# google/speedy

Measured on AMD Instinct MI355X. Metric: Msamples/s processed (16 kHz mono, 3.5x nonlinear), higher is better.
Workload: dtype int16 samples; f64 DFT, f32 features, int32 AMDF/OLA

## Files before the change

include/speedy_hip.h:

```cpp
#ifndef SPEEDY_HIP_H_
#define SPEEDY_HIP_H_
#include <stddef.h>
#include <stdint.h>
#ifdef __cplusplus
extern "C" {
#endif

#ifndef SPX_FEATURE_COUNT
#define SPX_FEATURE_COUNT 15
#endif

typedef struct spx_plan* spx_plan_t;

typedef struct {
  int64_t in_off;
  int64_t n_in;
  int64_t out_off;
  int64_t out_cap;
  int32_t channels;
  float speed;
  float nonlinear;
  float feedback;
} spx_stream_job;

// ... 52 lines not shown
void* spx_host_alloc(size_t bytes);
void spx_host_free(void* p);

int spx_batch_analyze(spx_plan_t plan, const spx_stream_job* jobs, int n_streams, const int16_t* in,
                      void* workspace, size_t workspace_bytes, const spx_taps* taps, void* hip_stream);
int spx_batch_walk(spx_plan_t plan, const spx_stream_job* jobs, int n_streams, const int16_t* in,
                   int16_t* out, int64_t* n_out, void* workspace, size_t workspace_bytes,
                   const spx_taps* taps, void* hip_stream);

size_t spx_batch_workspace_bytes_mixed(const spx_plan_t* plans, int n_plans, const spx_stream_job* jobs,
                                       const int* plan_index, int n_streams);
int spx_batch_run_mixed(const spx_plan_t* plans, int n_plans, const spx_stream_job* jobs, const int* plan_index,
                        int n_streams, const int16_t* in, int16_t* out, int64_t* n_out, void* workspace,
                        size_t workspace_bytes, void* hip_stream);

int spx_batch_run_mixed_taps(const spx_plan_t* plans, int n_plans, const spx_stream_job* jobs, const int* plan_index,
                             int n_streams, const int16_t* in, int16_t* out, int64_t* n_out, void* workspace,
                             size_t workspace_bytes, const spx_taps* taps, void* hip_stream);
int spx_batch_run_mixed_ahead(const spx_plan_t* plans, int n_plans, const spx_stream_job* jobs, const int* plan_index,
                              int n_streams, const int16_t* in, int16_t* out, int64_t* n_out, void* workspace,
                              size_t workspace_bytes, void* hip_stream);

void spx_set_timing(int enabled);
void spx_set_pipeline_chunks(int chunks);
void spx_set_concurrent(int on);
int spx_timing_collect(double* sum_ms_analyze, double* sum_ms_walk, int* n_calls);
const char* spx_batch_kernel_names(spx_plan_t plan, int n_streams, int max_channels, int speedup_only);
const char* spx_batch_kernel_names_lean(spx_plan_t plan, int n_streams, int max_channels, int speedup_only);
int spx_debug_last_walk_form(void);
int spx_debug_kernel_vgprs(int which);
int spx_debug_walk_info(int sample_rate, int channels, int n_streams, int speedup_only, int short_jobs, int lean, int* out5);
int spx_debug_analysis_info(int sample_rate, int* out4);
int spx_debug_mode_resources(int sample_rate, int channels, int n_streams, int speedup_only, long long* out22);
long long spx_debug_fdiv_check(unsigned seed, unsigned denominators, int exp_lo, int exp_hi);
long long spx_debug_xfade_check(int n_lo, int n_hi);
long long spx_debug_arith_check(unsigned seed, unsigned threads, unsigned per_thread);
int spx_debug_log_check(unsigned first_block, unsigned end_block, unsigned long long* sums);
int spx_debug_last_call_concurrent(void);
double spx_timing_last_tension_ms(void);

int spx_batch_read_steps(spx_plan_t plan, const spx_stream_job* jobs, int n_streams, const void* workspace,
                         int32_t* steps, void* hip_stream);
int spx_batch_read_steps_mixed(const spx_plan_t* plans, int n_plans, const spx_stream_job* jobs, const int* plan_index,
                               int n_streams, const void* workspace, int32_t* steps, void* hip_stream);

void* spx_device_alloc(size_t bytes);
void spx_device_free(void* p);
int spx_batch_pack_outputs(const spx_stream_job* jobs, int n_streams, const int16_t* out, const int64_t* n_out,
                           int16_t* packed, int64_t* offsets, void* hip_stream);
int spx_copy_to_device(void* dst, const void* src, size_t bytes, void* hip_stream);
int spx_copy_to_host(void* dst, const void* src, size_t bytes, void* hip_stream);
int spx_stream_synchronize(void* hip_stream);

#ifdef __cplusplus
}
#endif
#endif
```

speedy_amd/_lib.py:

```python
import ctypes as C
import os
import subprocess

_HERE = os.path.dirname(os.path.abspath(__file__))
LIB_PATH = os.environ.get("SPEEDY_HIP_LIB") or os.path.join(_HERE, "lib", "libspeedy_hip.so")
_LIB = None

c_short_p = C.POINTER(C.c_short)
c_float_p = C.POINTER(C.c_float)
c_int64_p = C.POINTER(C.c_int64)


class StreamJob(C.Structure):
    _fields_ = [("in_off", C.c_int64), ("n_in", C.c_int64), ("out_off", C.c_int64), ("out_cap", C.c_int64),
                ("channels", C.c_int32), ("speed", C.c_float), ("nonlinear", C.c_float), ("feedback", C.c_float)]


class Taps(C.Structure):
    _fields_ = [("tension", C.c_void_p), ("speed", C.c_void_p), ("features", C.c_void_p),
                ("spectrogram", C.c_void_p), ("normalized", C.c_void_p)]


TENSION_FN = C.CFUNCTYPE(None, C.c_void_p, C.c_int, C.c_float)
FEATURES_FN = C.CFUNCTYPE(None, C.c_void_p, C.c_int, c_float_p)
# ... 21 lines not shown
    "spx_batch_run_ahead_when": (C.c_int, [C.c_void_p, C.POINTER(StreamJob), C.c_int, C.c_void_p, C.c_void_p, C.c_void_p,
                                           C.c_void_p, C.c_size_t, C.POINTER(Taps), C.c_void_p, C.c_void_p]),
    "spx_batch_workspace_bytes_mixed": (C.c_size_t, [C.POINTER(C.c_void_p), C.c_int, C.POINTER(StreamJob), C.POINTER(C.c_int), C.c_int]),
    "spx_batch_run_mixed": (C.c_int, [C.POINTER(C.c_void_p), C.c_int, C.POINTER(StreamJob), C.POINTER(C.c_int), C.c_int,
                                      C.c_void_p, C.c_void_p, C.c_void_p, C.c_void_p, C.c_size_t, C.c_void_p]),
    "spx_batch_run_mixed_ahead": (C.c_int, [C.POINTER(C.c_void_p), C.c_int, C.POINTER(StreamJob), C.POINTER(C.c_int), C.c_int,
                                      C.c_void_p, C.c_void_p, C.c_void_p, C.c_void_p, C.c_size_t, C.c_void_p]),
    "spx_batch_run_mixed_taps": (C.c_int, [C.POINTER(C.c_void_p), C.c_int, C.POINTER(StreamJob), C.POINTER(C.c_int), C.c_int,
                                           C.c_void_p, C.c_void_p, C.c_void_p, C.c_void_p, C.c_size_t, C.POINTER(Taps), C.c_void_p]),
    "spx_batch_read_steps": (C.c_int, [C.c_void_p, C.POINTER(StreamJob), C.c_int, C.c_void_p, C.POINTER(C.c_int32), C.c_void_p]),
    "spx_batch_read_steps_mixed": (C.c_int, [C.POINTER(C.c_void_p), C.c_int, C.POINTER(StreamJob), C.POINTER(C.c_int), C.c_int,
                                             C.c_void_p, C.POINTER(C.c_int32), C.c_void_p]),
    "spx_batch_analyze": (C.c_int, [C.c_void_p, C.POINTER(StreamJob), C.c_int, C.c_void_p, C.c_void_p,
                                    C.c_size_t, C.POINTER(Taps), C.c_void_p]),
    "spx_batch_walk": (C.c_int, [C.c_void_p, C.POINTER(StreamJob), C.c_int, C.c_void_p, C.c_void_p, C.c_void_p,
                                 C.c_void_p, C.c_size_t, C.POINTER(Taps), C.c_void_p]),
    "spx_set_timing": (None, [C.c_int]),
    "spx_set_pipeline_chunks": (None, [C.c_int]),
    "spx_set_concurrent": (None, [C.c_int]),
    "spx_timing_collect": (C.c_int, [C.POINTER(C.c_double), C.POINTER(C.c_double), C.POINTER(C.c_int)]),
    "spx_timing_last_tension_ms": (C.c_double, []),
    "spx_batch_kernel_names": (C.c_char_p, [C.c_void_p, C.c_int, C.c_int, C.c_int]),
    "spx_batch_kernel_names_lean": (C.c_char_p, [C.c_void_p, C.c_int, C.c_int, C.c_int]),
    "spx_debug_last_walk_form": (C.c_int, []),
    "spx_debug_kernel_vgprs": (C.c_int, [C.c_int]),
    "spx_debug_last_call_concurrent": (C.c_int, []),
    "spx_debug_fdiv_check": (C.c_longlong, [C.c_uint, C.c_uint, C.c_int, C.c_int]),
    "spx_debug_xfade_check": (C.c_longlong, [C.c_int, C.c_int]),
    "spx_debug_arith_check": (C.c_longlong, [C.c_uint, C.c_uint, C.c_uint]),
    "spx_debug_log_check": (C.c_int, [C.c_uint, C.c_uint, C.POINTER(C.c_ulonglong)]),
    "spx_debug_walk_info": (C.c_int, [C.c_int, C.c_int, C.c_int, C.c_int, C.c_int, C.c_int, C.POINTER(C.c_int)]),
    "spx_debug_analysis_info": (C.c_int, [C.c_int, C.POINTER(C.c_int)]),
    "spx_debug_mode_resources": (C.c_int, [C.c_int, C.c_int, C.c_int, C.c_int, C.POINTER(C.c_longlong)]),
    "spx_pipeline_create": (C.c_void_p, [C.c_void_p, C.POINTER(StreamJob), C.c_int, C.c_int, C.c_uint]),
    "spx_pipeline_create_mixed": (C.c_void_p, [C.POINTER(C.c_void_p), C.c_int, C.POINTER(StreamJob), C.POINTER(C.c_int), C.c_int, C.c_int, C.c_uint]),
    "spx_pipeline_destroy": (None, [C.c_void_p]),
    "spx_pipeline_depth": (C.c_int, [C.c_void_p]),
    "spx_pipeline_input_values": (C.c_size_t, [C.c_void_p]),
    "spx_pipeline_host_input": (C.c_void_p, [C.c_void_p]),
    "spx_pipeline_submit": (C.c_int64, [C.c_void_p, C.c_void_p, C.c_int]),
    "spx_pipeline_input_consumed": (C.c_int, [C.c_void_p, C.c_int64]),
    "spx_pipeline_wait": (C.c_int, [C.c_void_p, C.c_int64, C.POINTER(C.c_void_p), C.POINTER(C.c_void_p), C.POINTER(C.c_void_p)]),
    "spx_host_alloc": (C.c_void_p, [C.c_size_t]),
    "spx_host_free": (None, [C.c_void_p]),
    "spx_device_alloc": (C.c_void_p, [C.c_size_t]),
    "spx_device_free": (None, [C.c_void_p]),
    "spx_copy_to_device": (C.c_int, [C.c_void_p, C.c_void_p, C.c_size_t, C.c_void_p]),
    "spx_copy_to_host": (C.c_int, [C.c_void_p, C.c_void_p, C.c_size_t, C.c_void_p]),
    "spx_batch_pack_outputs": (C.c_int, [C.c_void_p, C.c_int, C.c_void_p, C.c_void_p, C.c_void_p, C.c_void_p, C.c_void_p]),
    "spx_stream_synchronize": (C.c_int, [C.c_void_p]),
    "sonicCreateStream": (C.c_void_p, [C.c_int, C.c_int]),
    "sonicDestroyStream": (None, [C.c_void_p]),
    "sonicWriteShortToStream": (C.c_int, [C.c_void_p, c_short_p, C.c_int]),
    "sonicReadShortFromStream": (C.c_int, [C.c_void_p, c_short_p, C.c_int]),
    "sonicWriteFloatToStream": (C.c_int, [C.c_void_p, c_float_p, C.c_int]),
    "sonicReadFloatFromStream": (C.c_int, [C.c_void_p, c_float_p, C.c_int]),
    "sonicSetRate": (None, [C.c_void_p, C.c_float]),
    "sonicSetSpeed": (None, [C.c_void_p, C.c_float]),
    "sonicFlushStream": (C.c_int, [C.c_void_p]),
    "sonicEnableNonlinearSpeedup": (None, [C.c_void_p, C.c_float]),
    "sonicSetDurationFeedbackStrength": (None, [C.c_void_p, C.c_float]),
    "getSonicBufferSize": (C.c_int, [C.c_void_p]),
    "sonicSpectrogramSize": (C.c_int, [C.c_void_p]),
    "sonicTensionCallback": (None, [C.c_void_p, TENSION_FN]),
    "getSonicTensionCallback": (C.c_void_p, [C.c_void_p]),
    "sonicSpeedCallback": (None, [C.c_void_p, TENSION_FN]),
# ... 90 lines not shown
```

speedy_amd/csrc/spx_analysis.hip:

```cpp
#include <stdlib.h>

#include "spx_internal.h"
#include "spx_walk_common.h"

#ifndef SPX_TF
#define SPX_TF 16
#endif

#ifdef SPX_STAMPS
__device__ unsigned long long g_spx_astamps[16];
#define ASTAMP_DECL unsigned long long as_last = __builtin_readcyclecounter(), as_acc[10] = {0,0,0,0,0,0,0,0,0,0};
#define ASTAMP(i) do { const unsigned long long t_ = __builtin_readcyclecounter(); as_acc[i] += t_ - as_last; as_last = t_; } while (0)
#define ASTAMP_FLUSH if (threadIdx.x == 0 && blockIdx.x == 7) for (int i_ = 0; i_ < 10; i_++) g_spx_astamps[i_] += as_acc[i_];
extern "C" void spx_debug_astamps(unsigned long long* out, int reset) {
  (void)hipMemcpyFromSymbol(out, HIP_SYMBOL(g_spx_astamps), sizeof(unsigned long long) * 16);
  if (reset) { unsigned long long z[16] = {0}; (void)hipMemcpyToSymbol(HIP_SYMBOL(g_spx_astamps), z, sizeof(z)); }
}
#else
#define ASTAMP_DECL
#define ASTAMP(i)
#define ASTAMP_FLUSH
#endif

#ifndef SPX_TF_SMALL
#define SPX_TF_SMALL 8
#endif
#define SPX_TF_TINY 4
int spx_analysis_tile_frames() { return SPX_TF; }
int spx_analysis_small_tile_frames() { return SPX_TF_SMALL; }
int spx_analysis_tiny_tile_frames() { return SPX_TF_TINY; }

#define SPX_CB 24
static __host__ __device__ constexpr int spx_mag_stride(int W) { return (W + 4) & ~3; }
static __host__ __device__ constexpr int spx_cb(int tf) { return tf <= 8 ? 2 * SPX_CB : SPX_CB; }
// ... 364 lines not shown
template <class T>
__device__ __forceinline__ const T* per_frame(const T* p) {
  asm volatile("" : "+s"(p));
  return p;
}
__device__ __forceinline__ double uniform_f64(double v) {
  return __longlong_as_double(((long long)__builtin_amdgcn_readfirstlane((int)(__double_as_longlong(v) >> 32)) << 32) |
                              (unsigned)__builtin_amdgcn_readfirstlane((int)__double_as_longlong(v)));
}

#ifdef SPX_PREEMPH_V1
#define SPX_WIN_SCALE 1.0f
__device__ __forceinline__ float spx_preemph_win_f32(double md, double mpd, float w) {
  const float x = (float)(md / 32768.0), xp = (float)(mpd / 32768.0);
  const float y = (float)(1.0 * (double)x - 0.97 * (double)xp);
  return y * w;
}
#else
#define SPX_WIN_SCALE 0x1p-15f
__device__ __forceinline__ float spx_preemph_win_f32(double md, double mpd, float w15) {
  const float yy = (float)(md - 0.97 * mpd);
  return yy * w15;
}
#endif
__device__ __forceinline__ double spx_preemph_win(double md, double mpd, float w) { return (double)spx_preemph_win_f32(md, mpd, w); }
__device__ __forceinline__ cplx packed_point(const short* fr, int n, int j, int prev0, float w0, float w1) {
  const int i0 = 2 * n;
  const int m0 = fr[i0], m1 = fr[i0 + 1];
  const int mp0 = (i0 > 0) ? (int)fr[i0 - 1] : ((j > 0) ? (int)fr[prev0] : 0);
  const double d0 = (double)m0;
  return {spx_preemph_win(d0, (double)mp0, w0 * SPX_WIN_SCALE), spx_preemph_win((double)m1, d0, w1 * SPX_WIN_SCALE)};
}

#ifndef SPX_AN_W_330
#define SPX_AN_W_330 3
#endif
#ifndef SPX_AN_W_BIG
#define SPX_AN_W_BIG 2
#endif
template <int TF, int WCT>
__global__ void __launch_bounds__(SPX_BLOCK, (WCT == 240 || WCT == 120 || WCT == 180) ? 4 : WCT == 330 ? SPX_AN_W_330 : (WCT == 661 || WCT == 720) ? SPX_AN_W_BIG : (WCT == 480 || WCT == 360) ? 2 : 1)
spx_analysis_kernel(SpxPlanDev P, const SpxStreamDev* __restrict__ streams, int n_streams,
                    const int16_t* __restrict__ in_base, SpxFrameRec* __restrict__ rec, SpxTapsDev taps,
                    const int* __restrict__ tile_order, int* tile_flags, const float* __restrict__ frames,
                    int frame_mode) {
  extern __shared__ __attribute__((aligned(16))) unsigned char lds[];
  const int W = WCT ? WCT : P.W, B = P.B, N = 2 * W;
  const int tid = threadIdx.x, lane = tid & 63, wave = tid >> 6;

  const int tile = tile_order ? tile_order[blockIdx.x] : (int)blockIdx.x;
  int lo = 0, hi = n_streams - 1;
  while (lo < hi) {
    int mid = (lo + hi + 1) >> 1;
    if (streams[mid].first_tile <= tile) lo = mid; else hi = mid - 1;
  }
  const SpxStreamDev S = streams[lo];
  const int T = S.n_frames;
  const int j0 = S.frame_begin + (tile - S.first_tile) * TF;
  const int j1 = min(j0 + TF, T);
  const int C = S.channels;
  const int16_t* __restrict__ in = in_base + S.in_off;

  double* work = reinterpret_cast<double*>(lds);
  const size_t wb = work_bytes(W, TF, WCT != 0, (WCT != 0) ? 4 : P.dft_waves);
  float* mags = reinterpret_cast<float*>(lds + wb);
  const size_t mags_b = (((size_t)(TF + 1) * spx_mag_stride(W) * sizeof(float)) + 15) & ~(size_t)15;
  float* fE = reinterpret_cast<float*>(lds + wb + mags_b);
  float* fThr = fE + (TF + 1);
  float* fInv = fThr + (TF + 1);
  const int MS = spx_mag_stride(W);

  const size_t small_b = (((size_t)3 * (TF + 1) * sizeof(float)) + 15) & ~(size_t)15;
  const double* ltw = P.tw;
  const double* ltw2 = P.tw2;
  short* smono = reinterpret_cast<short*>(lds + wb + mags_b + small_b);

  double* bufA = work + (size_t)wave * (WCT != 0 ? 2 : 4) * W;
  double* bufB = (WCT != 0) ? bufA : bufA + 2 * W;

  const int jfirst = (j0 > 0) ? j0 - 1 : 0;
  const int64_t sbase = (int64_t)jfirst * B;
  const int nstage = (j1 - jfirst) * B + (W - B);
  if (frames != nullptr) {
  } else if (C == 1) {
    const int16_t* __restrict__ src = in + sbase;
    for (int k0 = tid; k0 < nstage; k0 += 8 * SPX_BLOCK) {
      short v[8];
#pragma unroll
      for (int u = 0; u < 8; u++) { const int k = k0 + u * SPX_BLOCK; v[u] = (k < nstage) ? src[k] : (short)0; }
#pragma unroll
      for (int u = 0; u < 8; u++) { const int k = k0 + u * SPX_BLOCK; if (k < nstage) smono[k] = v[u]; }
    }
  } else {
    for (int k = tid; k < nstage; k += SPX_BLOCK) smono[k] = (short)mono_sample(in, sbase + k, C);
  }
  __syncthreads();

  ASTAMP_DECL
  if constexpr (WCT == 240) {
    const double2* twp = reinterpret_cast<const double2*>(P.tw);
    const double2* tw2p = reinterpret_cast<const double2*>(P.tw2);
    const int b = lane;
    const bool on60 = b < 60, on48 = b < 48;
    const int bb = on60 ? b : 0;
    double2 w1[3], w2[3], w3[2][2], wu[4];
    float wn[4];
#pragma unroll
    for (int j = 1; j < 4; j++) { w1[j - 1] = twp[bb * j]; w2[j - 1] = twp[4 * (bb >> 2) * j]; }
#pragma unroll
    for (int u = 0; u < 2; u++) {
      const int b3 = lane + 64 * u, p3 = (b3 < 80) ? (b3 >> 4) : 0;
      w3[u][0] = twp[16 * p3];
      w3[u][1] = twp[32 * p3];
    }
#pragma unroll
    for (int u = 0; u < 4; u++) { const int k = lane + 64 * u; wu[u] = tw2p[k < 240 ? k : 0]; }
    wn[0] = P.window[2 * bb]; wn[1] = P.window[2 * bb + 1]; wn[2] = P.window[2 * bb + 120]; wn[3] = P.window[2 * bb + 121];
#pragma unroll
    for (int k = 0; k < 4; k++) wn[k] *= SPX_WIN_SCALE;
    for (int s = wave; s <= TF; s += 4) {
      const int j = j0 - 1 + s;
      float* mrow = mags + (size_t)s * MS;
      if (j < 0 || j >= j1) {
        for (int k = lane; k < 240; k += SPX_WAVE) mrow[k] = 0.0f;
        continue;
      }
      const short* fr = smono + (size_t)(j - jfirst) * B;
      if (on60) {
        const int i0 = 2 * b, i1 = 2 * b + 120;
        const int m0 = fr[i0], m1 = fr[i0 + 1], m2 = fr[i1], m3 = fr[i1 + 1];
        const int mp0 = (i0 > 0) ? (int)fr[i0 - 1] : ((j > 0) ? (int)fr[(240 - B) - 1] : 0);
        const int mp2 = fr[i1 - 1];
        const double d0 = (double)m0, d2 = (double)m2;
        const cplx a0 = {spx_preemph_win(d0, (double)mp0, wn[0]), spx_preemph_win((double)m1, d0, wn[1])},
                   a1 = {spx_preemph_win(d2, (double)mp2, wn[2]), spx_preemph_win((double)m3, d2, wn[3])};
        const cplx b0 = {a0.r + a1.r, a0.i + a1.i}, b2 = {a0.r - a1.r, a0.i - a1.i};
        const cplx b1 = {a0.r + a1.i, a0.i - a1.r}, b3 = {a0.r - a1.i, a0.i + a1.r};
        st(bufA, 4 * b, b0);
        st(bufA, 4 * b + 1, cmul_tw(b1, w1[0]));
        st(bufA, 4 * b + 2, cmul_tw(b2, w1[1]));
        st(bufA, 4 * b + 3, cmul_tw(b3, w1[2]));
      }
      wave_sync();
      ASTAMP(0);
      if (on60) {
        const cplx a0 = ld(bufA, b), a1 = ld(bufA, b + 60), a2 = ld(bufA, b + 120), a3 = ld(bufA, b + 180);
        wave_sync();
        const cplx t0 = {a0.r + a2.r, a0.i + a2.i}, t1 = {a0.r - a2.r, a0.i - a2.i};
        const cplx t2 = {a1.r + a3.r, a1.i + a3.i}, t3 = {a1.r - a3.r, a1.i - a3.i};
        const cplx b0 = {t0.r + t2.r, t0.i + t2.i}, b2 = {t0.r - t2.r, t0.i - t2.i};
        const cplx b1 = {t1.r + t3.i, t1.i - t3.r}, b3 = {t1.r - t3.i, t1.i + t3.r};
        const int o = (b & 3) + 16 * (b >> 2);
        st(bufB, o, b0);
// ... 19 lines not shown
            const cplx t2 = {spx_bf3h(a0.r, t1.r), spx_bf3h(a0.i, t1.i)};
            const cplx t3 = {S3_1 * (a1.r - a2.r), S3_1 * (a1.i - a2.i)};
            const cplx b0 = {a0.r + t1.r, a0.i + t1.i};
            const cplx b1 = {t2.r + t3.i, t2.i - t3.r}, b2 = {t2.r - t3.i, t2.i + t3.r};
            const int o = (b3i & 15) + 48 * (b3i >> 4);
            st(bufA, o, b0);
            st(bufA, o + 16, cmul_tw(b1, w3[u][0]));
            st(bufA, o + 32, cmul_tw(b2, w3[u][1]));
          }
        }
      }
      wave_sync();
      if (on48) {
        const cplx a0 = ld(bufA, b), a1 = ld(bufA, b + 48), a2 = ld(bufA, b + 96), a3 = ld(bufA, b + 144),
                   a4 = ld(bufA, b + 192);
        wave_sync();
        const cplx t1 = {a1.r + a4.r, a1.i + a4.i}, t2 = {a2.r + a3.r, a2.i + a3.i};
        const cplx t3 = {a1.r - a4.r, a1.i - a4.i}, t4 = {a2.r - a3.r, a2.i - a3.i};
        const cplx b0 = {(a0.r + t1.r) + t2.r, (a0.i + t1.i) + t2.i};
        const cplx m1 = {spx_bf5m(a0.r, C5_1, t1.r, C5_2, t2.r), spx_bf5m(a0.i, C5_1, t1.i, C5_2, t2.i)};
        const cplx m2 = {spx_bf5m(a0.r, C5_2, t1.r, C5_1, t2.r), spx_bf5m(a0.i, C5_2, t1.i, C5_1, t2.i)};
        const cplx n1 = {spx_bf5n(S5_1, t3.r, S5_2, t4.r), spx_bf5n(S5_1, t3.i, S5_2, t4.i)};
        const cplx n2 = {spx_bf5d(S5_2, t3.r, S5_1, t4.r), spx_bf5d(S5_2, t3.i, S5_1, t4.i)};
        const cplx b1 = {m1.r + n1.i, m1.i - n1.r}, b4 = {m1.r - n1.i, m1.i + n1.r};
        const cplx b2 = {m2.r + n2.i, m2.i - n2.r}, b3 = {m2.r - n2.i, m2.i + n2.r};
        st(bufB, b, b0);
        st(bufB, b + 48, b1);
        st(bufB, b + 96, b2);
        st(bufB, b + 144, b3);
        st(bufB, b + 192, b4);
      }
      wave_sync();
      ASTAMP(1);
      float* spec_out = taps.spectrogram ? taps.spectrogram + (size_t)(S.frame_off + j) * 480 : nullptr;
#pragma unroll
      for (int u = 0; u < 4; u++) {
        const int k = lane + 64 * u;
        if (k < 240) {
          const int k2 = (k == 0) ? 0 : 240 - k;
          const cplx a = ld(bufB, k), c = ld(bufB, k2);
          const double b_r = c.r, b_i = -c.i;
          const float mag = spx_untangle_mag(a.r, a.i, b_r, b_i, wu[u]);
          mrow[k] = mag;
          if (spec_out) {
            spec_out[k] = mag;
            if (k > 0) spec_out[480 - k] = mag;
            else spec_out[240] = (float)__builtin_fabs(a.r - a.i);
          }
        }
      }
      wave_sync();
      ASTAMP(2);
    }
  } else if constexpr (WCT == 330) {
    const double2* twp = reinterpret_cast<const double2*>(P.tw);
    const double2* tw2p = reinterpret_cast<const double2*>(P.tw2);
    double2 w1[3], w2[2][2];
    float wn[3][2];
#pragma unroll
    for (int u = 0; u < 3; u++) {
      const int b1 = (lane + 64 * u < 165) ? lane + 64 * u : 0;
      w1[u] = twp[b1];
      wn[u][0] = P.window[2 * b1] * SPX_WIN_SCALE; wn[u][1] = P.window[2 * b1 + 1] * SPX_WIN_SCALE;
    }
#pragma unroll
    for (int u = 0; u < 2; u++) {
      const int p2 = (lane + 64 * u < 110) ? ((lane + 64 * u) >> 1) : 0;
      w2[u][0] = twp[2 * p2];
      w2[u][1] = twp[4 * p2];
    }
    double wc[10], ws[10];
#pragma unroll
    for (int k = 1; k <= 10; k++) {
      const double2 w = twp[k * 30];
      wc[k - 1] = __longlong_as_double(((long long)__builtin_amdgcn_readfirstlane((int)(__double_as_longlong(w.x) >> 32)) << 32) |
                                       (unsigned)__builtin_amdgcn_readfirstlane((int)__double_as_longlong(w.x)));
      ws[k - 1] = __longlong_as_double(((long long)__builtin_amdgcn_readfirstlane((int)(__double_as_longlong(w.y) >> 32)) << 32) |
                                       (unsigned)__builtin_amdgcn_readfirstlane((int)__double_as_longlong(w.y)));
    }
    for (int s = wave; s <= TF; s += 4) {
      const int j = j0 - 1 + s;
      float* mrow = mags + (size_t)s * MS;
      if (j < 0 || j >= j1) {
        for (int k = lane; k < 330; k += SPX_WAVE) mrow[k] = 0.0f;
        continue;
      }
      const short* fr = smono + (size_t)(j - jfirst) * B;
#pragma unroll
      for (int u = 0; u < 3; u++) {
        const int b = lane + 64 * u;
        if (b < 165) {
          const int i0 = 2 * b;
          const int m0 = fr[i0], m1 = fr[i0 + 1];
          const int mp0 = (i0 > 0) ? (int)fr[i0 - 1] : ((j > 0) ? (int)fr[(330 - B) - 1] : 0);
          const double d0 = (double)m0;
          const cplx a0 = {spx_preemph_win(d0, (double)mp0, wn[u][0]), spx_preemph_win((double)m1, d0, wn[u][1])};
          st(bufA, 2 * b, a0);
          st(bufA, 2 * b + 1, cmul_tw(a0, w1[u]));
        }
      }
      wave_sync();
      ASTAMP(0);
      {
        cplx q0[2], q1[2], q2[2];
#pragma unroll
        for (int u = 0; u < 2; u++) {
          const int b = (lane + 64 * u < 110) ? lane + 64 * u : 0;
          q0[u] = ld(bufA, b); q1[u] = ld(bufA, b + 110); q2[u] = ld(bufA, b + 220);
        }
        wave_sync();
#pragma unroll
        for (int u = 0; u < 2; u++) {
          const int b = lane + 64 * u;
// ... 363 lines not shown
#ifdef SPX_ROWMAX_V1
    for (int s = wave - 1; s <= TF; s += 3) {
      const float* mrow = mags + (size_t)s * MS;
      float mx = 0.0f;
      for (int i = 1 + lane; i < W; i += SPX_WAVE) mx = fmaxf(mx, mrow[i]);
#pragma unroll
      for (int d = 32; d >= 1; d >>= 1) mx = fmaxf(mx, __shfl_xor(mx, d));
      if (lane == 0) fThr[s] = (float)((double)mx / 100.0);
    }
#else
    unsigned keep = 0u;
    int nrows = 0;
    for (int s = wave - 1; s <= TF; s += 3, nrows++) {
      const unsigned* mrow = reinterpret_cast<const unsigned*>(mags + (size_t)s * MS);
      unsigned m = 0u;
      for (int q = lane; 4 * q < W; q += SPX_WAVE) {
        const uint4 v = *reinterpret_cast<const uint4*>(mrow + 4 * q);
        const unsigned a = (q == 0) ? 0u : v.x;
        const unsigned b = (4 * q + 1 < W) ? v.y : 0u, c = (4 * q + 2 < W) ? v.z : 0u, d = (4 * q + 3 < W) ? v.w : 0u;
        const unsigned ab = a > b ? a : b, cd = c > d ? c : d;
        const unsigned abcd = ab > cd ? ab : cd;
        m = m > abcd ? m : abcd;
      }
      const float mx = wave_max_f(__builtin_bit_cast(float, m));
      if (lane == nrows) keep = __builtin_bit_cast(unsigned, mx);
    }
    if (lane < nrows) fThr[wave - 1 + 3 * lane] = (float)((double)__builtin_bit_cast(float, keep) / 100.0);
#endif
#ifndef SPX_LOG_V1
    if (tid < SPX_WAVE + 128)
      reinterpret_cast<uint4*>(reinterpret_cast<unsigned char*>(work) + terms_bytes(W, TF, WCT != 0))[tid - SPX_WAVE] =
          reinterpret_cast<const uint4*>(spx_log_table_dev)[tid - SPX_WAVE];
#endif
  } else if (tid <= TF) {
    const float4* r4 = reinterpret_cast<const float4*>(mags + (size_t)tid * MS);
    float e = 0.0f;
    __builtin_amdgcn_s_setprio(3);
    auto acc8 = [&](const float4& p, const float4& q) {
      const float4 pp = {p.x * p.x, p.y * p.y, p.z * p.z, p.w * p.w}, qq = {q.x * q.x, q.y * q.y, q.z * q.z, q.w * q.w};
      e += pp.x; e += pp.y; e += pp.z; e += pp.w;
      e += qq.x; e += qq.y; e += qq.z; e += qq.w;
    };
    {
      const float4 h = r4[0];
      if (1 < W) e += h.y * h.y;
      if (2 < W) e += h.z * h.z;
      if (3 < W) e += h.w * h.w;
    }
    int i = 4;
    float4 c0 = r4[1], c1 = r4[2], c2 = r4[3], c3 = r4[4];
#pragma unroll 1
    for (; i + 16 <= W; i += 16) {
      const float4 n0 = r4[(i >> 2) + 4], n1 = r4[(i >> 2) + 5], n2 = r4[(i >> 2) + 6], n3 = r4[(i >> 2) + 7];
      __builtin_amdgcn_sched_barrier(0);
      acc8(c0, c1);
      acc8(c2, c3);
      c0 = n0; c1 = n1; c2 = n2; c3 = n3;
    }
    {
      const float t[16] = {c0.x, c0.y, c0.z, c0.w, c1.x, c1.y, c1.z, c1.w, c2.x, c2.y, c2.z, c2.w, c3.x, c3.y, c3.z, c3.w};
#pragma unroll
      for (int u = 0; u < 16; u++)
        if (i + u < W) e += t[u] * t[u];
    }
    __builtin_amdgcn_s_setprio(0);
    const float eps = 2.2204e-16f;
    fE[tid] = e;
// ... 153 lines not shown
    const int f = idx / (W - 1);
    const int i = 1 + (idx - f * (W - 1));
    terms[(size_t)f * (W + 1) + i] = log_term(f, i);
  }
  __syncthreads();
  ASTAMP(6);

  if (tid < nfr) {
    const double* trow = terms + (size_t)tid * (W + 1);
    float lsd = 0.0f;
    int i = 1;
    for (; i + 8 <= W; i += 8) {
      double tv[8];
#pragma unroll
      for (int u = 0; u < 8; u++) tv[u] = trow[i + u];
#pragma unroll
      for (int u = 0; u < 8; u++) lsd = (float)((double)lsd + tv[u]);
    }
    for (; i < W; i++) lsd = (float)((double)lsd + trow[i]);
    write_rec(tid, lsd);
  }
  }
  if (tile_flags) {
    asm volatile("s_waitcnt vmcnt(0)" ::: "memory");
    __syncthreads();
    if (tid == 0) {
      __builtin_amdgcn_fence(__ATOMIC_RELEASE, "agent");
      asm volatile("s_waitcnt vmcnt(0)" ::: "memory");
      __hip_atomic_store(&tile_flags[tile], 1, __ATOMIC_RELAXED, __HIP_MEMORY_SCOPE_AGENT);
    }
  }
  ASTAMP(7);
  ASTAMP_FLUSH
}

__global__ void spx_arith_check_kernel(unsigned seed, unsigned per_thread, unsigned long long* bad) {
  unsigned long long st = (unsigned long long)seed * 0x9E3779B97F4A7C15ull + (blockIdx.x * blockDim.x + threadIdx.x) * 0xD1B54A32D192ED03ull + 1;
  auto next = [&]() { st ^= st >> 12; st ^= st << 25; st ^= st >> 27; return st * 0x2545F4914F6CDD1Dull; };
  unsigned long long miss = 0;
  for (unsigned i = 0; i < per_thread; i++) {
    const unsigned long long a = next(), b = next(), c = next();
    const float fn = __uint_as_float((unsigned)((127 - 53 + (a % 57)) << 23) | (unsigned)((a >> 8) & 0x7fffff));
    const float fd = __uint_as_float((unsigned)((127 - 53 + (b % 57)) << 23) | (unsigned)((b >> 8) & 0x7fffff));
    if (__float_as_uint(spx_fdiv32(fn, fd)) != __float_as_uint(fn / fd)) miss++;
    const long long fb = ((long long)(1023 - 21 + (c % 20)) << 52) | (long long)((c >> 8) & 0xfffffffffffffll) | ((c >> 63) ? (1ll << 63) : 0);
    const double f = __longlong_as_double(fb);
    if (__double_as_longlong(spx_fdiv64(f, 2.0 + f)) != __double_as_longlong(f / (2.0 + f))) miss++;
    const long long xb = ((long long)(1023 - 800 + (a >> 33) % 1811) << 52) | (long long)((b >> 10) & 0xfffffffffffffll);
    const double x = ((c & 1023) == 0) ? 0.0 : __longlong_as_double(xb);
    if (__float_as_uint(spx_sqrt64_to_f32(x)) != __float_as_uint((float)__builtin_sqrt(x))) miss++;
  }
  if (miss) atomicAdd(bad, miss);
}
extern "C" long long spx_debug_arith_check(unsigned seed, unsigned threads, unsigned per_thread) {
  unsigned long long* d = nullptr;
  unsigned long long h = 0;
  if (hipMalloc(&d, sizeof(h)) != hipSuccess) return -1;
  if (hipMemcpy(d, &h, sizeof(h), hipMemcpyHostToDevice) != hipSuccess) { (void)hipFree(d); return -1; }
  const unsigned blocks = (threads + 255) / 256;
  hipLaunchKernelGGL(spx_arith_check_kernel, dim3(blocks), dim3(256), 0, nullptr, seed, per_thread, d);
  const bool ok = hipDeviceSynchronize() == hipSuccess && hipMemcpy(&h, d, sizeof(h), hipMemcpyDeviceToHost) == hipSuccess;
  (void)hipFree(d);
  return ok ? (long long)h : -1;
}

__global__ void __launch_bounds__(256) spx_log_check_kernel(unsigned first_block, unsigned long long* __restrict__ sums) {
// ... 2 lines not shown
  __shared__ unsigned long long acc;
  if (threadIdx.x < 128) reinterpret_cast<uint4*>(tab)[threadIdx.x] = reinterpret_cast<const uint4*>(spx_log_table_dev)[threadIdx.x];
  if (threadIdx.x == 0) acc = 0;
  __syncthreads();
  const unsigned b = first_block + blockIdx.x;
  unsigned long long sum = 0;
  for (unsigned i = threadIdx.x; i < (1u << 20); i += 256) {
    const float x = __uint_as_float((b << 20) | i);
    sum += (unsigned long long)__double_as_longlong(spx_log_v2_f32(x, tab));
  }
  atomicAdd(&acc, sum);
  __syncthreads();
  if (threadIdx.x == 0) sums[b] = acc;
#endif
}
extern "C" int spx_debug_log_check(unsigned first_block, unsigned end_block, unsigned long long* sums) {
#ifdef SPX_LOG_V1
  (void)first_block; (void)end_block; (void)sums;
  return -3;
#else
  if (first_block < 8) first_block = 8;
  if (end_block > 2040) end_block = 2040;
  if (!sums || first_block >= end_block) return -1;
  unsigned long long* d = nullptr;
  if (hipMalloc(&d, 2040 * sizeof(unsigned long long)) != hipSuccess) return -1;
  bool ok = hipMemset(d, 0, 2040 * sizeof(unsigned long long)) == hipSuccess;
  if (ok) hipLaunchKernelGGL(spx_log_check_kernel, dim3(end_block - first_block), dim3(256), 0, nullptr, first_block, d);
  ok = ok && hipDeviceSynchronize() == hipSuccess && hipMemcpy(sums, d, 2040 * sizeof(unsigned long long), hipMemcpyDeviceToHost) == hipSuccess;
  (void)hipFree(d);
  return ok ? 0 : -1;
#endif
}

void spx_launch_analysis(const SpxPlanDev& P, const SpxStreamDev* streams, int n_streams, int n_tiles,
                         const int16_t* in, SpxFrameRec* rec, SpxTapsDev taps, const int* tile_order, int* tile_flags,
                         hipStream_t st) {
  if (n_tiles <= 0) return;
  const size_t lds = spx_analysis_lds_bytes(P);
  const int ctw = plan_ct_window(P);
#define SPX_LAUNCH_ANALYSIS(TFV, WV)                                                                                   \
  hipLaunchKernelGGL((spx_analysis_kernel<TFV, WV>), dim3(n_tiles), dim3(SPX_BLOCK), lds, st, P, streams, n_streams, in, \
                     rec, taps, tile_order, tile_flags, (const float*)nullptr, 0)
  if (P.tile_frames == SPX_TF_TINY) {
    SPX_LAUNCH_ANALYSIS(SPX_TF_TINY, 0);
  } else if (P.tile_frames == SPX_TF_SMALL) {
    if (ctw == 240) SPX_LAUNCH_ANALYSIS(SPX_TF_SMALL, 240); else if (ctw == 330) SPX_LAUNCH_ANALYSIS(SPX_TF_SMALL, 330);
    else if (ctw == 720) SPX_LAUNCH_ANALYSIS(SPX_TF_SMALL, 720); else if (ctw == 661) SPX_LAUNCH_ANALYSIS(SPX_TF_SMALL, 661);
    else if (ctw == 120) SPX_LAUNCH_ANALYSIS(SPX_TF_SMALL, 120);
    else SPX_LAUNCH_ANALYSIS(SPX_TF_SMALL, 0);
  } else {
    if (ctw == 240) SPX_LAUNCH_ANALYSIS(SPX_TF, 240); else if (ctw == 330) SPX_LAUNCH_ANALYSIS(SPX_TF, 330);
    else if (ctw == 120) SPX_LAUNCH_ANALYSIS(SPX_TF, 120); else if (ctw == 360) SPX_LAUNCH_ANALYSIS(SPX_TF, 360);
    else if (ctw == 180) SPX_LAUNCH_ANALYSIS(SPX_TF, 180);
    else if (ctw == 480) SPX_LAUNCH_ANALYSIS(SPX_TF, 480);
    else SPX_LAUNCH_ANALYSIS(SPX_TF, 0);
  }
#undef SPX_LAUNCH_ANALYSIS
}

int spx_analysis_vgprs(const SpxPlanDev& P, int* scratch_bytes) {
  const int ctw = plan_ct_window(P);
  const bool small = P.tile_frames == SPX_TF_SMALL;
  const void* fn;
#define SPX_AN_FN(TFV, WV) reinterpret_cast<const void*>(spx_analysis_kernel<TFV, WV>)
  if (P.tile_frames == SPX_TF_TINY) fn = SPX_AN_FN(SPX_TF_TINY, 0);
  else if (small) fn = ctw == 240 ? SPX_AN_FN(SPX_TF_SMALL, 240) : ctw == 330 ? SPX_AN_FN(SPX_TF_SMALL, 330)
                     : ctw == 720 ? SPX_AN_FN(SPX_TF_SMALL, 720) : ctw == 661 ? SPX_AN_FN(SPX_TF_SMALL, 661)
                     : ctw == 120 ? SPX_AN_FN(SPX_TF_SMALL, 120) : SPX_AN_FN(SPX_TF_SMALL, 0);
  else fn = ctw == 240 ? SPX_AN_FN(SPX_TF, 240) : ctw == 330 ? SPX_AN_FN(SPX_TF, 330) : ctw == 120 ? SPX_AN_FN(SPX_TF, 120)
          : ctw == 360 ? SPX_AN_FN(SPX_TF, 360) : ctw == 480 ? SPX_AN_FN(SPX_TF, 480) : ctw == 180 ? SPX_AN_FN(SPX_TF, 180)
          : SPX_AN_FN(SPX_TF, 0);
#undef SPX_AN_FN
  return spx_kernel_vgprs(fn, scratch_bytes);
}

void spx_launch_analysis_frames(const SpxPlanDev& P, const SpxStreamDev* streams, int n_tiles, const float* frames,
                                bool preemph, SpxFrameRec* rec, SpxTapsDev taps, hipStream_t st) {
  if (n_tiles <= 0) return;
  SpxPlanDev Q = P;
  if (Q.tile_frames != SPX_TF_SMALL && Q.tile_frames != SPX_TF_TINY) Q.tile_frames = SPX_TF;
  const size_t lds = analysis_lds_bytes(Q, false);
  if (Q.tile_frames == SPX_TF_TINY)
    hipLaunchKernelGGL((spx_analysis_kernel<SPX_TF_TINY, 0>), dim3(n_tiles), dim3(SPX_BLOCK), lds, st, Q, streams, 1,
                       (const int16_t*)nullptr, rec, taps, (const int*)nullptr, (int*)nullptr, frames, preemph ? 1 : 2);
  else if (Q.tile_frames == SPX_TF_SMALL)
    hipLaunchKernelGGL((spx_analysis_kernel<SPX_TF_SMALL, 0>), dim3(n_tiles), dim3(SPX_BLOCK), lds, st, Q, streams, 1,
                       (const int16_t*)nullptr, rec, taps, (const int*)nullptr, (int*)nullptr, frames, preemph ? 1 : 2);
  else
    hipLaunchKernelGGL((spx_analysis_kernel<SPX_TF, 0>), dim3(n_tiles), dim3(SPX_BLOCK), lds, st, Q, streams, 1,
                       (const int16_t*)nullptr, rec, taps, (const int*)nullptr, (int*)nullptr, frames, preemph ? 1 : 2);
}
```

speedy_amd/csrc/spx_mode_table.cpp:

```cpp
#include <string.h>

#include "spx_mode.h"

#define SPX_Q_FIELDS(X)                                                                                                         \
  X(n) X(max_channels) X(do_a) X(do_w) X(has_frames) X(forced) X(force_concurrent) X(force_ahead) X(force_total_streams)        \
  X(ahead_req) X(overlap_req) X(cu_count) X(lds_per_cu) X(walk_lds) X(walk_waves) X(walk_vgprs) X(walk_fast) X(walk_nwc)        \
  X(lean_lds) X(lean_waves) X(lean_vgprs) X(lean_fast) X(lean_nwc) X(lean_valid) X(tension_lds) X(tension_vgprs)                \
  X(tile_default) X(tile_big) X(tile_small) X(an_lds_default) X(an_lds_small) X(an_vgprs_default) X(an_vgprs_small)             \
  X(concurrent_enabled) X(chunks_set) X(chunks) X(trial_state_key) X(trial_calls) X(trial_choice) X(two_workspaces)            \
  X(guard_busy) X(trial_times_ready) X(us_seq) X(us_con) X(trial_key) X(device_ours)
#define SPX_A_FIELDS(X)                                                                                                         \
  X(lean_walk) X(launch_lean) X(tile_frames) X(co_resident) X(doubtful) X(trial_slot) X(want_concurrent) X(concurrent)          \
  X(ahead) X(seq_ahead) X(ahead_forced) X(walk2) X(nch) X(exclusive_cu) X(asked_device) X(next_key) X(next_calls) X(next_choice)

enum {
#define X(f) Q_##f,
  SPX_Q_FIELDS(X)
#undef X
  Q_COUNT
};
enum {
#define X(f) A_##f,
  SPX_A_FIELDS(X)
#undef X
  A_COUNT
};

static bool ours_cb(void* ctx) { return *static_cast<long long*>(ctx) != 0; }

extern "C" {
const char* spx_mode_table_query_fields(void) {
  return
#define X(f) #f " "
      SPX_Q_FIELDS(X)
// ... 33 lines not shown
  T.device_ours = ours_cb; T.device_ctx = &ours;
  const SpxMode M = spx_choose_mode(S, R, E, T, trial);
  a[A_lean_walk] = M.lean_walk; a[A_launch_lean] = M.launch_lean; a[A_tile_frames] = M.tile_frames; a[A_co_resident] = M.co_resident;
  a[A_doubtful] = M.doubtful; a[A_trial_slot] = M.trial_slot; a[A_want_concurrent] = M.want_concurrent; a[A_concurrent] = M.concurrent;
  a[A_ahead] = M.ahead; a[A_seq_ahead] = M.seq_ahead; a[A_ahead_forced] = M.ahead_forced; a[A_walk2] = M.walk2; a[A_nch] = M.nch;
  a[A_exclusive_cu] = M.exclusive_cu; a[A_asked_device] = M.asked_device; a[A_next_key] = M.trial_next.key;
  a[A_next_calls] = M.trial_next.calls; a[A_next_choice] = M.trial_next.choice;
  return 0;
}
int spx_mode_table_mixed_mode(const long long* groups, int n_groups, int n_total, int cu_count, long long lds_per_cu, long long tension_lds,
                              int tension_vgprs, int concurrent_enabled, int ahead_req, int guard_busy, int device_ours, long long* out4) {
  SpxModeGroup G[8];
  if (n_groups < 0 || n_groups > 8) return -1;
  for (int g = 0; g < n_groups; g++) {
    const long long* p = groups + 7 * g;
    G[g].n = (int)p[0];
    G[g].walk = {(size_t)p[1], (int)p[2], (int)p[3], true, 4};
    G[g].any_nonlinear = p[4] != 0;
    G[g].an_lds = (size_t)p[5];
    G[g].an_vgprs = (int)p[6];
  }
  SpxModeEnv E;
  memset(&E, 0, sizeof(E));
  E.concurrent_enabled = concurrent_enabled; E.chunks = 1;
  SpxModeRuntime T;
  memset(&T, 0, sizeof(T));
  long long ours = device_ours;
  T.guard_busy = guard_busy; T.device_ours = ours_cb; T.device_ctx = &ours;
  const SpxMixedMode M = spx_choose_mixed_mode(G, n_groups, n_total, cu_count, (size_t)lds_per_cu, (size_t)tension_lds, tension_vgprs, E,
                                               ahead_req != 0, T);
  out4[0] = M.concurrent; out4[1] = M.ahead; out4[2] = M.chain_analyses; out4[3] = M.asked_device;
  return 0;
}
int spx_mode_table_mixed_walk2(int concurrent, int ahead, int detached, int taps) {
  SpxMixedMode M = {concurrent != 0, ahead != 0, false, false};
  return spx_mixed_walk2(M, detached != 0, taps != 0) ? 1 : 0;
}
}
```

Baseline: 45620.

## Process runs of consecutive analysis tiles per block, reusing the overlap frame

```diff
diff --git a/include/speedy_hip.h b/include/speedy_hip.h
--- a/include/speedy_hip.h
+++ b/include/speedy_hip.h
@@ -108,6 +108,7 @@
 int spx_debug_walk_info(int sample_rate, int channels, int n_streams, int speedup_only, int short_jobs, int lean, int* out5);
 int spx_debug_analysis_info(int sample_rate, int* out4);
 int spx_debug_mode_resources(int sample_rate, int channels, int n_streams, int speedup_only, long long* out22);
+int spx_debug_set_analysis_run(int run_tiles);
 long long spx_debug_fdiv_check(unsigned seed, unsigned denominators, int exp_lo, int exp_hi);
 long long spx_debug_xfade_check(int n_lo, int n_hi);
 long long spx_debug_arith_check(unsigned seed, unsigned threads, unsigned per_thread);
diff --git a/speedy_amd/_lib.py b/speedy_amd/_lib.py
--- a/speedy_amd/_lib.py
+++ b/speedy_amd/_lib.py
@@ -77,6 +77,7 @@
     "spx_debug_walk_info": (C.c_int, [C.c_int, C.c_int, C.c_int, C.c_int, C.c_int, C.c_int, C.POINTER(C.c_int)]),
     "spx_debug_analysis_info": (C.c_int, [C.c_int, C.POINTER(C.c_int)]),
     "spx_debug_mode_resources": (C.c_int, [C.c_int, C.c_int, C.c_int, C.c_int, C.POINTER(C.c_longlong)]),
+    "spx_debug_set_analysis_run": (C.c_int, [C.c_int]),
     "spx_pipeline_create": (C.c_void_p, [C.c_void_p, C.POINTER(StreamJob), C.c_int, C.c_int, C.c_uint]),
     "spx_pipeline_create_mixed": (C.c_void_p, [C.POINTER(C.c_void_p), C.c_int, C.POINTER(StreamJob), C.POINTER(C.c_int), C.c_int, C.c_int, C.c_uint]),
     "spx_pipeline_destroy": (None, [C.c_void_p]),
diff --git a/speedy_amd/csrc/spx_an_run.h b/speedy_amd/csrc/spx_an_run.h
--- /dev/null
+++ b/speedy_amd/csrc/spx_an_run.h
@@ -0,0 +1,19 @@
+#pragma once
+
+#ifndef SPX_AN_RUN
+#define SPX_AN_RUN 4
+#endif
+#define SPX_AN_RUN_MAX 64
+
+static inline int spx_an_run_length(int ct_window, int tile_frames, int default_tile, bool ordered, int requested) {
+  if (ordered) return 1;
+  if (tile_frames != default_tile || ct_window != 240) return 1;
+  int r = requested > 0 ? requested : SPX_AN_RUN;
+  if (r > SPX_AN_RUN_MAX) r = SPX_AN_RUN_MAX;
+  return r < 1 ? 1 : r;
+}
+static inline int spx_an_grid(int n_tiles, int run) {
+  if (n_tiles <= 0) return 0;
+  if (run < 1) run = 1;
+  return (n_tiles + run - 1) / run;
+}
diff --git a/speedy_amd/csrc/spx_analysis.hip b/speedy_amd/csrc/spx_analysis.hip
--- a/speedy_amd/csrc/spx_analysis.hip
+++ b/speedy_amd/csrc/spx_analysis.hip
@@ -1,5 +1,8 @@
 #include <stdlib.h>
 
+#include <atomic>
+
+#include "spx_an_run.h"
 #include "spx_internal.h"
 #include "spx_walk_common.h"
 
@@ -430,6 +433,60 @@
   return {spx_preemph_win(d0, (double)mp0, w0 * SPX_WIN_SCALE), spx_preemph_win((double)m1, d0, w1 * SPX_WIN_SCALE)};
 }
 
+template <int WCT> struct an_lane_consts {
+  __device__ __forceinline__ void load(const SpxPlanDev&, int) {}
+};
+template <> struct an_lane_consts<240> {
+  double2 w1[3], w2[3], w3[2][2], wu[4];
+  float wn[4];
+  __device__ __forceinline__ void load(const SpxPlanDev& P, const int lane) {
+    const double2* twp = reinterpret_cast<const double2*>(P.tw);
+    const double2* tw2p = reinterpret_cast<const double2*>(P.tw2);
+    const int bb = lane < 60 ? lane : 0;
+#pragma unroll
+    for (int j = 1; j < 4; j++) { w1[j - 1] = twp[bb * j]; w2[j - 1] = twp[4 * (bb >> 2) * j]; }
+#pragma unroll
+    for (int u = 0; u < 2; u++) {
+      const int b3 = lane + 64 * u, p3 = (b3 < 80) ? (b3 >> 4) : 0;
+      w3[u][0] = twp[16 * p3];
+      w3[u][1] = twp[32 * p3];
+    }
+#pragma unroll
+    for (int u = 0; u < 4; u++) { const int k = lane + 64 * u; wu[u] = tw2p[k < 240 ? k : 0]; }
+    wn[0] = P.window[2 * bb]; wn[1] = P.window[2 * bb + 1]; wn[2] = P.window[2 * bb + 120]; wn[3] = P.window[2 * bb + 121];
+#pragma unroll
+    for (int k = 0; k < 4; k++) wn[k] *= SPX_WIN_SCALE;
+  }
+};
+template <> struct an_lane_consts<330> {
+  double2 w1[3], w2[2][2];
+  float wn[3][2];
+  double wc[10], ws[10];
+  __device__ __forceinline__ void load(const SpxPlanDev& P, const int lane) {
+    const double2* twp = reinterpret_cast<const double2*>(P.tw);
+#pragma unroll
+    for (int u = 0; u < 3; u++) {
+      const int b1 = (lane + 64 * u < 165) ? lane + 64 * u : 0;
+      w1[u] = twp[b1];
+      wn[u][0] = P.window[2 * b1] * SPX_WIN_SCALE; wn[u][1] = P.window[2 * b1 + 1] * SPX_WIN_SCALE;
+    }
+#pragma unroll
+    for (int u = 0; u < 2; u++) {
+      const int p2 = (lane + 64 * u < 110) ? ((lane + 64 * u) >> 1) : 0;
+      w2[u][0] = twp[2 * p2];
+      w2[u][1] = twp[4 * p2];
+    }
+#pragma unroll
+    for (int k = 1; k <= 10; k++) {
+      const double2 w = twp[k * 30];
+      wc[k - 1] = uniform_f64(w.x);
+      ws[k - 1] = uniform_f64(w.y);
+    }
+  }
+};
+
+template <int TF, int WCT> struct an_runs { static constexpr bool value = TF == SPX_TF && WCT == 240; };
+
 #ifndef SPX_AN_W_330
 #define SPX_AN_W_330 3
 #endif
@@ -441,16 +498,31 @@
 spx_analysis_kernel(SpxPlanDev P, const SpxStreamDev* __restrict__ streams, int n_streams,
                     const int16_t* __restrict__ in_base, SpxFrameRec* __restrict__ rec, SpxTapsDev taps,
                     const int* __restrict__ tile_order, int* tile_flags, const float* __restrict__ frames,
-                    int frame_mode) {
+                    int frame_mode, int n_tiles, int run) {
   extern __shared__ __attribute__((aligned(16))) unsigned char lds[];
   const int W = WCT ? WCT : P.W, B = P.B, N = 2 * W;
-  const int tid = threadIdx.x, lane = tid & 63, wave = tid >> 6;
-
-  const int tile = tile_order ? tile_order[blockIdx.x] : (int)blockIdx.x;
-  int lo = 0, hi = n_streams - 1;
-  while (lo < hi) {
-    int mid = (lo + hi + 1) >> 1;
-    if (streams[mid].first_tile <= tile) lo = mid; else hi = mid - 1;
+  constexpr bool RUNS = an_runs<TF, WCT>::value;
+
+  const int runl = RUNS ? run : 1;
+  const int tile_begin = tile_order ? tile_order[blockIdx.x] : (int)blockIdx.x * runl;
+  const int nsub = RUNS ? min(runl, n_tiles - tile_begin) : 1;
+  int lo = 0;
+  for (int sub = 0; sub < nsub; sub++) {
+  int tid = threadIdx.x;
+  if constexpr (RUNS) {
+    asm volatile("" : "+v"(tid));
+    __builtin_assume(tid >= 0 && tid < SPX_BLOCK);
+  }
+  const int lane = tid & 63, wave = tid >> 6;
+  const int tile = tile_begin + sub;
+  const bool carried = RUNS && sub > 0 && (lo == n_streams - 1 || streams[lo + 1].first_tile > tile);
+  if (!carried) {
+    int hi = n_streams - 1;
+    lo = 0;
+    while (lo < hi) {
+      int mid = (lo + hi + 1) >> 1;
+      if (streams[mid].first_tile <= tile) lo = mid; else hi = mid - 1;
+    }
   }
   const SpxStreamDev S = streams[lo];
   const int T = S.n_frames;
@@ -458,6 +530,7 @@
   const int j1 = min(j0 + TF, T);
   const int C = S.channels;
   const int16_t* __restrict__ in = in_base + S.in_off;
+  const int s0 = carried ? 1 : 0;
 
   double* work = reinterpret_cast<double*>(lds);
   const size_t wb = work_bytes(W, TF, WCT != 0, (WCT != 0) ? 4 : P.dft_waves);
@@ -476,7 +549,12 @@
   double* bufA = work + (size_t)wave * (WCT != 0 ? 2 : 4) * W;
   double* bufB = (WCT != 0) ? bufA : bufA + 2 * W;
 
-  const int jfirst = (j0 > 0) ? j0 - 1 : 0;
+  if (carried && wave == 3) {
+    for (int q = lane; 4 * q < W; q += SPX_WAVE)
+      reinterpret_cast<float4*>(mags)[q] = reinterpret_cast<const float4*>(mags + (size_t)TF * MS)[q];
+    if (lane == 0) { fE[0] = fE[TF]; fInv[0] = fInv[TF]; }
+  }
+  const int jfirst = carried ? j0 : (j0 > 0) ? j0 - 1 : 0;
   const int64_t sbase = (int64_t)jfirst * B;
   const int nstage = (j1 - jfirst) * B + (W - B);
   if (frames != nullptr) {
@@ -495,28 +573,13 @@
   __syncthreads();
 
   ASTAMP_DECL
+  an_lane_consts<WCT> K;
+  K.load(P, lane);
   if constexpr (WCT == 240) {
-    const double2* twp = reinterpret_cast<const double2*>(P.tw);
-    const double2* tw2p = reinterpret_cast<const double2*>(P.tw2);
     const int b = lane;
     const bool on60 = b < 60, on48 = b < 48;
-    const int bb = on60 ? b : 0;
-    double2 w1[3], w2[3], w3[2][2], wu[4];
-    float wn[4];
-#pragma unroll
-    for (int j = 1; j < 4; j++) { w1[j - 1] = twp[bb * j]; w2[j - 1] = twp[4 * (bb >> 2) * j]; }
-#pragma unroll
-    for (int u = 0; u < 2; u++) {
-      const int b3 = lane + 64 * u, p3 = (b3 < 80) ? (b3 >> 4) : 0;
-      w3[u][0] = twp[16 * p3];
-      w3[u][1] = twp[32 * p3];
-    }
-#pragma unroll
-    for (int u = 0; u < 4; u++) { const int k = lane + 64 * u; wu[u] = tw2p[k < 240 ? k : 0]; }
-    wn[0] = P.window[2 * bb]; wn[1] = P.window[2 * bb + 1]; wn[2] = P.window[2 * bb + 120]; wn[3] = P.window[2 * bb + 121];
-#pragma unroll
-    for (int k = 0; k < 4; k++) wn[k] *= SPX_WIN_SCALE;
-    for (int s = wave; s <= TF; s += 4) {
+    const auto& w1 = K.w1; const auto& w2 = K.w2; const auto& w3 = K.w3; const auto& wu = K.wu; const auto& wn = K.wn;
+    for (int s = s0 + wave; s <= TF; s += 4) {
       const int j = j0 - 1 + s;
       float* mrow = mags + (size_t)s * MS;
       if (j < 0 || j >= j1) {
@@ -602,6 +665,7 @@
       }
       wave_sync();
       ASTAMP(1);
+      const double2* tw2q = per_frame(reinterpret_cast<const double2*>(P.tw2));
       float* spec_out = taps.spectrogram ? taps.spectrogram + (size_t)(S.frame_off + j) * 480 : nullptr;
 #pragma unroll
       for (int u = 0; u < 4; u++) {
@@ -610,7 +674,7 @@
           const int k2 = (k == 0) ? 0 : 240 - k;
           const cplx a = ld(bufB, k), c = ld(bufB, k2);
           const double b_r = c.r, b_i = -c.i;
-          const float mag = spx_untangle_mag(a.r, a.i, b_r, b_i, wu[u]);
+          const float mag = spx_untangle_mag(a.r, a.i, b_r, b_i, RUNS ? tw2q[k] : wu[u]);
           mrow[k] = mag;
           if (spec_out) {
             spec_out[k] = mag;
@@ -625,30 +689,8 @@
   } else if constexpr (WCT == 330) {
     const double2* twp = reinterpret_cast<const double2*>(P.tw);
     const double2* tw2p = reinterpret_cast<const double2*>(P.tw2);
-    double2 w1[3], w2[2][2];
-    float wn[3][2];
-#pragma unroll
-    for (int u = 0; u < 3; u++) {
-      const int b1 = (lane + 64 * u < 165) ? lane + 64 * u : 0;
-      w1[u] = twp[b1];
-      wn[u][0] = P.window[2 * b1] * SPX_WIN_SCALE; wn[u][1] = P.window[2 * b1 + 1] * SPX_WIN_SCALE;
-    }
-#pragma unroll
-    for (int u = 0; u < 2; u++) {
-      const int p2 = (lane + 64 * u < 110) ? ((lane + 64 * u) >> 1) : 0;
-      w2[u][0] = twp[2 * p2];
-      w2[u][1] = twp[4 * p2];
-    }
-    double wc[10], ws[10];
-#pragma unroll
-    for (int k = 1; k <= 10; k++) {
-      const double2 w = twp[k * 30];
-      wc[k - 1] = __longlong_as_double(((long long)__builtin_amdgcn_readfirstlane((int)(__double_as_longlong(w.x) >> 32)) << 32) |
-                                       (unsigned)__builtin_amdgcn_readfirstlane((int)__double_as_longlong(w.x)));
-      ws[k - 1] = __longlong_as_double(((long long)__builtin_amdgcn_readfirstlane((int)(__double_as_longlong(w.y) >> 32)) << 32) |
-                                       (unsigned)__builtin_amdgcn_readfirstlane((int)__double_as_longlong(w.y)));
-    }
-    for (int s = wave; s <= TF; s += 4) {
+    const auto& w1 = K.w1; const auto& w2 = K.w2; const auto& wn = K.wn; const auto& wc = K.wc; const auto& ws = K.ws;
+    for (int s = s0 + wave; s <= TF; s += 4) {
       const int j = j0 - 1 + s;
       float* mrow = mags + (size_t)s * MS;
       if (j < 0 || j >= j1) {
@@ -1078,7 +1120,7 @@
       reinterpret_cast<uint4*>(reinterpret_cast<unsigned char*>(work) + terms_bytes(W, TF, WCT != 0))[tid - SPX_WAVE] =
           reinterpret_cast<const uint4*>(spx_log_table_dev)[tid - SPX_WAVE];
 #endif
-  } else if (tid <= TF) {
+  } else if (tid >= s0 && tid <= TF) {
     const float4* r4 = reinterpret_cast<const float4*>(mags + (size_t)tid * MS);
     float e = 0.0f;
     __builtin_amdgcn_s_setprio(3);
@@ -1298,6 +1340,7 @@
   }
   ASTAMP(7);
   ASTAMP_FLUSH
+  }
 }
 
 __global__ void spx_arith_check_kernel(unsigned seed, unsigned per_thread, unsigned long long* bad) {
@@ -1366,15 +1409,23 @@
 #endif
 }
 
+static std::atomic<int> g_an_run{0};
+extern "C" int spx_debug_set_analysis_run(int run) {
+  g_an_run.store(run < 0 ? 0 : run, std::memory_order_relaxed);
+  return spx_an_run_length(240, SPX_TF, SPX_TF, false, g_an_run.load(std::memory_order_relaxed));
+}
+
 void spx_launch_analysis(const SpxPlanDev& P, const SpxStreamDev* streams, int n_streams, int n_tiles,
                          const int16_t* in, SpxFrameRec* rec, SpxTapsDev taps, const int* tile_order, int* tile_flags,
                          hipStream_t st) {
   if (n_tiles <= 0) return;
   const size_t lds = spx_analysis_lds_bytes(P);
   const int ctw = plan_ct_window(P);
+  const int run = spx_an_run_length(ctw, P.tile_frames, SPX_TF, tile_order != nullptr, g_an_run.load(std::memory_order_relaxed));
+  const int grid = spx_an_grid(n_tiles, run);
 #define SPX_LAUNCH_ANALYSIS(TFV, WV)                                                                                   \
-  hipLaunchKernelGGL((spx_analysis_kernel<TFV, WV>), dim3(n_tiles), dim3(SPX_BLOCK), lds, st, P, streams, n_streams, in, \
-                     rec, taps, tile_order, tile_flags, (const float*)nullptr, 0)
+  hipLaunchKernelGGL((spx_analysis_kernel<TFV, WV>), dim3(grid), dim3(SPX_BLOCK), lds, st, P, streams, n_streams, in,   \
+                     rec, taps, tile_order, tile_flags, (const float*)nullptr, 0, n_tiles, run)
   if (P.tile_frames == SPX_TF_TINY) {
     SPX_LAUNCH_ANALYSIS(SPX_TF_TINY, 0);
   } else if (P.tile_frames == SPX_TF_SMALL) {
@@ -1416,11 +1467,14 @@
   const size_t lds = analysis_lds_bytes(Q, false);
   if (Q.tile_frames == SPX_TF_TINY)
     hipLaunchKernelGGL((spx_analysis_kernel<SPX_TF_TINY, 0>), dim3(n_tiles), dim3(SPX_BLOCK), lds, st, Q, streams, 1,
-                       (const int16_t*)nullptr, rec, taps, (const int*)nullptr, (int*)nullptr, frames, preemph ? 1 : 2);
+                       (const int16_t*)nullptr, rec, taps, (const int*)nullptr, (int*)nullptr, frames, preemph ? 1 : 2,
+                       n_tiles, 1);
   else if (Q.tile_frames == SPX_TF_SMALL)
     hipLaunchKernelGGL((spx_analysis_kernel<SPX_TF_SMALL, 0>), dim3(n_tiles), dim3(SPX_BLOCK), lds, st, Q, streams, 1,
-                       (const int16_t*)nullptr, rec, taps, (const int*)nullptr, (int*)nullptr, frames, preemph ? 1 : 2);
+                       (const int16_t*)nullptr, rec, taps, (const int*)nullptr, (int*)nullptr, frames, preemph ? 1 : 2,
+                       n_tiles, 1);
   else
     hipLaunchKernelGGL((spx_analysis_kernel<SPX_TF, 0>), dim3(n_tiles), dim3(SPX_BLOCK), lds, st, Q, streams, 1,
-                       (const int16_t*)nullptr, rec, taps, (const int*)nullptr, (int*)nullptr, frames, preemph ? 1 : 2);
-}
+                       (const int16_t*)nullptr, rec, taps, (const int*)nullptr, (int*)nullptr, frames, preemph ? 1 : 2,
+                       n_tiles, 1);
+}
diff --git a/speedy_amd/csrc/spx_mode_table.cpp b/speedy_amd/csrc/spx_mode_table.cpp
--- a/speedy_amd/csrc/spx_mode_table.cpp
+++ b/speedy_amd/csrc/spx_mode_table.cpp
@@ -1,5 +1,6 @@
 #include <string.h>
 
+#include "spx_an_run.h"
 #include "spx_mode.h"
 
 #define SPX_Q_FIELDS(X)                                                                                                         \
@@ -99,6 +100,11 @@
   out4[0] = M.concurrent; out4[1] = M.ahead; out4[2] = M.chain_analyses; out4[3] = M.asked_device;
   return 0;
 }
+int spx_mode_table_analysis_run(int ct_window, int tile_frames, int default_tile, int ordered, int requested) {
+  return spx_an_run_length(ct_window, tile_frames, default_tile, ordered != 0, requested);
+}
+int spx_mode_table_analysis_grid(int n_tiles, int run) { return spx_an_grid(n_tiles, run); }
+int spx_mode_table_analysis_run_shipped(void) { return SPX_AN_RUN; }
 int spx_mode_table_mixed_walk2(int concurrent, int ahead, int detached, int taps) {
   SpxMixedMode M = {concurrent != 0, ahead != 0, false, false};
   return spx_mixed_walk2(M, detached != 0, taps != 0) ? 1 : 0;
```

Result: slower. 44620 (-2.2%).
